# darren-huang/SmartStartContinuous

Measured on NVIDIA B200. Metric: mpc_rollout_steps_per_s, higher is better.
Workload: dtype bf16 (tcgen05, fp32 accumulate; first/last layer, state, scoring fp32)

## Files before the change

### smartstartcontinuous_b200/csrc/mpc_tc.cu

```cuda
#include <cuda_bf16.h>

#include <cstdlib>
#include <cstring>

#include "mpc_kernels.cuh"
#include "tc_ptx.cuh"
#include "tc_score_row.cuh"

namespace tc {

constexpr int TM = 128;
constexpr int NC = 128;
constexpr int NH = NC / 2;
constexpr int KSLAB = 256;
constexpr int STAGE_BYTES = NH * KSLAB * 2;
constexpr int NSTAGE = 4;
constexpr int K1_MAX = 32;
constexpr int ACC_SLOTS = 2;
constexpr int W1_CHUNK_BYTES_MAX = NH * K1_MAX * 2;
constexpr int A1_BYTES_MAX = TM * K1_MAX * 2;
constexpr int ROW_WARPS = 8;
constexpr int TPR = ROW_WARPS / 4;
constexpr int CPT = NC / TPR;
constexpr int ROW_THREADS = ROW_WARPS * 32;
constexpr int THREADS = ROW_THREADS + 64;
constexpr int HP_MAX = 512;
constexpr int MAX_DIN = (K1_MAX - 2) / 3;
__host__ __device__ constexpr int dz_of(int d) { return d <= 2 ? 2 : (d <= 3 ? 3 : (d <= 4 ? 4 : 8)); }
__host__ __device__ constexpr int k1_slots(int d, int da) { return 3 * (dz_of(d) + da) + 2 <= 16 ? 16 : 32; }
__host__ __device__ constexpr int w3_pair_floats(int dz) { return dz <= 2 ? 4 : (dz <= 4 ? 8 : 16); }
constexpr uint32_t TMEM_COLS = 512;
constexpr uint32_t COL_H1 = 0, COL_ACC = 256;
constexpr int CLUSTER = 2;

struct Params {
    const __nv_bfloat16* w1_img;
    const __nv_bfloat16* w2_img;
    const float* w3;
    const float* b3;
    int hp;
    int din;
    long long tile_begin, tile_end;
    int iters;
    unsigned long long* prof;
};

constexpr uint32_t IDESC = (1u << 4) | (1u << 7) | (1u << 10) | ((uint32_t)(NC >> 3) << 17) |
                           ((uint32_t)((2 * TM) >> 4) << 24);


#define TC_TRACE(ev)                                                                              \
    do {                                                                                          \
        if (p.prof && blockIdx.x == 0 && lane == 0 && trace_it == 0 && trace_t >= 10 && trace_t < 13) \
            trace_s[(trace_t - 10) * 256 + (ev)] = (unsigned long long)clock64();                  \
    } while (0)

template <int DZ>
struct SmemT {
    static constexpr size_t W2_RING = 0;
    static constexpr size_t W1 = W2_RING + (size_t)NSTAGE * STAGE_BYTES;
    static constexpr size_t A1 = W1 + (size_t)(HP_MAX / NC) * W1_CHUNK_BYTES_MAX;
    static constexpr size_t W3 = A1 + (size_t)A1_BYTES_MAX;
    static constexpr size_t ZX = W3 + (size_t)(HP_MAX / 2) * w3_pair_floats(DZ) * 4;
    static constexpr size_t BARS = ZX + (size_t)TPR * TM * 8 * 4;
    static constexpr int N_BARS = 3 * NSTAGE + 2 * ACC_SLOTS + 2 * (HP_MAX / NC) + 2;
    static constexpr size_t TMEM_PTR = BARS + (size_t)N_BARS * 8;
    static constexpr size_t TRACE = TMEM_PTR + 16;
    static constexpr size_t END = TRACE;
};

template <int DT, int DZ, int K1T>
__global__ void __launch_bounds__(THREADS, 1) mpc_rollout_tc_kernel(const RolloutArgs a, const Params p) {
    pdl_trigger();
    extern __shared__ __align__(128) unsigned char smem[];
    using Smem = SmemT<DZ>;
    constexpr int MAXIN = (K1T - 2) / 3;
    constexpr int W1_CHUNK_BYTES = NH * K1T * 2;
    constexpr int DZP = w3_pair_floats(DZ) / 2;
    unsigned char* w2_ring = smem + Smem::W2_RING;
    unsigned char* w1s = smem + Smem::W1;
    unsigned char* a1s = smem + Smem::A1;
    float* w3s = reinterpret_cast<float*>(smem + Smem::W3);
    float* zx = reinterpret_cast<float*>(smem + Smem::ZX);
    uint64_t* bars = reinterpret_cast<uint64_t*>(smem + Smem::BARS);
    uint64_t* w2_full = bars;
    uint64_t* w2_peer = w2_full + NSTAGE;
    uint64_t* w2_empty = w2_peer + NSTAGE;
    uint64_t* acc_full = w2_empty + NSTAGE;
    uint64_t* acc_free = acc_full + ACC_SLOTS;
    uint64_t* h1_ready = acc_free + ACC_SLOTS;
    uint64_t* l1_full = h1_ready + HP_MAX / NC;
    uint64_t* x_ready = l1_full + HP_MAX / NC;
    uint64_t* w1_full = x_ready + 1;
    uint32_t* tmem_ptr = reinterpret_cast<uint32_t*>(smem + Smem::TMEM_PTR);

    const int tid = threadIdx.x, warp = tid >> 5, lane = tid & 31;
    const int T = a.H + 1;
    unsigned long long* trace_s = reinterpret_cast<unsigned long long*>(smem + Smem::TRACE);
    if (p.prof && blockIdx.x == 0)
        for (int i = tid; i < 3 * 256; i += THREADS) trace_s[i] = 0;
    unsigned long long trace_clk0 = 0, trace_ns0 = 0;
    if (p.prof && blockIdx.x == 0 && tid == 0) {
        trace_clk0 = (unsigned long long)clock64();
        asm volatile("mov.u64 %0, %%globaltimer;" : "=l"(trace_ns0));
    }
    const int nch = p.hp / NC;
    const int nslab = p.hp / KSLAB;
    static_assert(KSLAB % NC == 0, "a K-slab covers whole layer-1 chunks");
    constexpr int CPS = KSLAB / NC;
    const uint32_t cta_rank = cluster_ctarank();
    const bool leader = cta_rank == 0;

    if (tid == 0) {
        for (int s = 0; s < NSTAGE; ++s) {
            mbar_init(&w2_full[s], leader ? 2 : 1);
            mbar_init(&w2_peer[s], 1);
            mbar_init(&w2_empty[s], 1);
        }
        for (int s = 0; s < ACC_SLOTS; ++s) { mbar_init(&acc_full[s], 1); mbar_init(&acc_free[s], 2 * ROW_WARPS); }
        for (int c = 0; c < HP_MAX / NC; ++c) { mbar_init(&h1_ready[c], 2 * ROW_WARPS); mbar_init(&l1_full[c], 1); }
        mbar_init(x_ready, 2 * 4);
        mbar_init(w1_full, 1);
        asm volatile("fence.mbarrier_init.release.cluster;" ::: "memory");
    }
    if (warp == 0) {
        asm volatile("tcgen05.alloc.cta_group::2.sync.aligned.shared::cta.b32 [%0], %1;" ::"r"(smem_u32(tmem_ptr)),
                     "n"(TMEM_COLS));
        asm volatile("tcgen05.relinquish_alloc_permit.cta_group::2.sync.aligned;");
    }
    for (int i = tid; i < (p.hp / 2) * (2 * DZP); i += THREADS) w3s[i] = p.w3[i];
    __syncthreads();
    if (tid == 0) {
        mbar_expect_tx(w1_full, (uint32_t)(nch * W1_CHUNK_BYTES));
        bulk_g2s(w1s, reinterpret_cast<const unsigned char*>(p.w1_img) + (size_t)cta_rank * nch * W1_CHUNK_BYTES,
                 (uint32_t)(nch * W1_CHUNK_BYTES), w1_full);
        mbar_wait<false>(w1_full, 0);
    }
    tc_fence_before();
    __syncthreads();
    cluster_sync_all();
    tc_fence_after();
    const uint32_t tmem = *tmem_ptr;

    if (warp < ROW_WARPS) {
        const int q = warp & 3, ch = warp >> 2;
        const int row = q * 32 + lane;
        const uint32_t lane_addr = tmem + ((uint32_t)(q * 32) << 16);
        uint32_t step_it = 0;
        float upd_s[DZ], upd_c[DZ];
#pragma unroll
        for (int j = 0; j < DZ; ++j) {
            upd_s[j] = j < a.d ? a.norm.std_z[j] : 0.f;
            upd_c[j] = j < a.d ? fmaf(__ldg(p.b3 + j), a.norm.std_z[j], a.norm.mean_z[j]) : 0.f;
            asm volatile("" : "+f"(upd_s[j]), "+f"(upd_c[j]));
        }
        for (int it = 0; it < p.iters; ++it) {
            const long long tile = p.tile_begin + (long long)it * gridDim.x + blockIdx.x;
            const long long k_local = tile * TM + row;
            const bool live = tile < p.tile_end && k_local < a.K_local;
            const long long n_qcols = 4 * ((a.K_local + TM - 1) / TM);
            const long long qcol = tile < p.tile_end ? tile * 4 + q : -1;
            float x[DT];
            ScoreAcc sc;
#pragma unroll
            for (int j = 0; j < DT; ++j) x[j] = j < a.d ? a.state0[j] : 0.f;
            if (ch == 1) score_init<DT>(a.plan, a.wp_index, x, sc);
            float act[SS_MAX_DA];
#pragma unroll
            for (int j = 0; j < SS_MAX_DA; ++j) act[j] = 0.f;
            ActionCursor cur;
            action_cursor_init(cur);
            if (ch == 0 && live) {
#pragma unroll
                for (int j = 0; j < SS_MAX_DA; ++j)
                    if (j < a.da) act[j] = fetch_action_seq(a.act, cur, k_local, a.k_offset + k_local, 0, j);
            }
            for (int t = 0; t < a.H; ++t, ++step_it) {
                const int trace_it = (warp == 0 || warp == 4) ? it : 1, trace_t = t;
                const int tb = warp == 4 ? 100 : 0;
                TC_TRACE(tb + 0);
                if (ch == 0) {
                    float xin[MAXIN];
#pragma unroll
                    for (int j = 0; j < MAXIN; ++j) xin[j] = 0.f;
#pragma unroll
                    for (int j = 0; j < DZ; ++j)
                        if (j < MAXIN) xin[j] = (x[j] - a.norm.mean_x[j]) * a.norm.inv_std_x[j];
#pragma unroll
                    for (int j = 0; j < SS_MAX_DA; ++j)
                        if (DZ + j < MAXIN) xin[DZ + j] = (act[j] - a.norm.mean_y[j]) * a.norm.inv_std_y[j];
                    float slot[K1T];
#pragma unroll
                    for (int s = 0; s < K1T; ++s) slot[s] = 0.f;
#pragma unroll
                    for (int j = 0; j < MAXIN; ++j) {
                        const float hi = bf16_hi(xin[j]);
                        const float lo = xin[j] - hi;
                        slot[3 * j] = hi;
                        slot[3 * j + 1] = hi;
                        slot[3 * j + 2] = lo;
                    }
                    slot[K1T - 2] = 1.f;
                    slot[K1T - 1] = 1.f;
#pragma unroll
                    for (int kc = 0; kc < K1T / 8; ++kc) {
                        uint4 v;
                        v.x = pack_bf16(slot[8 * kc], slot[8 * kc + 1]);
                        v.y = pack_bf16(slot[8 * kc + 2], slot[8 * kc + 3]);
                        v.z = pack_bf16(slot[8 * kc + 4], slot[8 * kc + 5]);
                        v.w = pack_bf16(slot[8 * kc + 6], slot[8 * kc + 7]);
                        *reinterpret_cast<uint4*>(a1s + kc * (TM * 16) + row * 16) = v;
                    }
                    TC_TRACE(60);
                    asm volatile("fence.proxy.async.shared::cta;" ::: "memory");
                    TC_TRACE(61);
                    __syncwarp();
                    if (lane == 0) mbar_arrive_leader(x_ready);
                }
                TC_TRACE(tb + 1);
                static_assert(CPT == 64, "two 32-column TMEM loads per thread and chunk");
                for (int c0 = 0; c0 < nch; c0 += 2) {
                    const uint32_t slot_i = (uint32_t)(c0 >> 1);
                    uint32_t v0[32], v1[32], pk0[16], pk1[16];
                    if (c0 == 0) mbar_wait<false>(&l1_full[0], step_it & 1);
                    TC_TRACE(tb + 2 + c0);
                    tc_fence_after();
                    tmem_ld32(lane_addr + COL_H1 + slot_i * NC + ch * CPT, v0);
                    tmem_ld32(lane_addr + COL_H1 + slot_i * NC + ch * CPT + 32, v1);
                    tmem_wait_ld();
                    asm volatile("bar.sync %0, 64;" ::"r"(2 + q) : "memory");
#pragma unroll
                    for (int c2 = 0; c2 < 16; ++c2) {
                        pk0[c2] = pack_bf16_relu(__uint_as_float(v0[2 * c2]), __uint_as_float(v0[2 * c2 + 1]));
                        pk1[c2] = pack_bf16_relu(__uint_as_float(v1[2 * c2]), __uint_as_float(v1[2 * c2 + 1]));
                    }
                    tmem_st16(lane_addr + COL_H1 + c0 * (NC / 2) + ch * (CPT / 2), pk0);
                    tmem_st16(lane_addr + COL_H1 + c0 * (NC / 2) + ch * (CPT / 2) + 16, pk1);
                    TC_TRACE(tb + 6 + c0);
                    if (c0 == 0) {
                        mbar_wait<false>(&l1_full[1], step_it & 1);
                        tc_fence_after();
                    }
                    TC_TRACE(tb + 3 + c0);
                    tmem_ld32(lane_addr + COL_ACC + slot_i * NC + ch * CPT, v0);
                    tmem_ld32(lane_addr + COL_ACC + slot_i * NC + ch * CPT + 32, v1);
                    tmem_wait_st();
                    tc_fence_before();
                    __syncwarp();
                    if (lane == 0) mbar_arrive_leader(&h1_ready[c0]);
                    tmem_wait_ld();
                    tc_fence_before();
                    __syncwarp();
                    if (lane == 0) mbar_arrive_leader(&acc_free[slot_i]);
#pragma unroll
                    for (int c2 = 0; c2 < 16; ++c2) {
                        pk0[c2] = pack_bf16_relu(__uint_as_float(v0[2 * c2]), __uint_as_float(v0[2 * c2 + 1]));
                        pk1[c2] = pack_bf16_relu(__uint_as_float(v1[2 * c2]), __uint_as_float(v1[2 * c2 + 1]));
                    }
                    tmem_st16(lane_addr + COL_H1 + (c0 + 1) * (NC / 2) + ch * (CPT / 2), pk0);
                    tmem_st16(lane_addr + COL_H1 + (c0 + 1) * (NC / 2) + ch * (CPT / 2) + 16, pk1);
                    tmem_wait_st();
                    tc_fence_before();
                    __syncwarp();
                    if (lane == 0) mbar_arrive_leader(&h1_ready[c0 + 1]);
                    TC_TRACE(tb + 7 + c0);
                }
                if (ch == 1) {
                    score_row<DT>(a, t, x, sc, live, k_local, qcol, n_qcols, lane);
                } else if (ch == 0 && live && t + 1 < a.H) {
                    TC_TRACE(70);
#pragma unroll
                    for (int j = 0; j < SS_MAX_DA; ++j)
                        if (j < a.da) act[j] = fetch_action_seq(a.act, cur, k_local, a.k_offset + k_local, t + 1, j);
                    TC_TRACE(71);
                }
                TC_TRACE(tb + 19);
                float2 zacc[DZ];
#pragma unroll
                for (int j = 0; j < DZ; ++j) zacc[j] = make_float2(0.f, 0.f);
                for (int n = 0; n < nch; ++n) {
                    const uint32_t slot_i = (uint32_t)(n & 1);
                    const uint32_t full_k = step_it * (uint32_t)((nch + 1 - (int)slot_i) >> 1) + (uint32_t)(n >> 1);
                    mbar_wait<false>(&acc_full[slot_i], full_k & 1);
                    TC_TRACE(tb + 10 + n);
                    tc_fence_after();
                    uint32_t v0[32], v1[32];
                    tmem_ld32(lane_addr + COL_ACC + slot_i * NC + ch * CPT, v0);
                    tmem_ld32(lane_addr + COL_ACC + slot_i * NC + ch * CPT + 32, v1);
                    tmem_wait_ld();
                    tc_fence_before();
                    __syncwarp();
                    if (lane == 0) mbar_arrive_leader(&acc_free[slot_i]);
                    const float* wrow = w3s + (size_t)((n * NC + ch * CPT) / 2) * (2 * DZP);
#pragma unroll
                    for (int j2 = 0; j2 < CPT / 2; ++j2) {
                        const uint32_t ua = j2 < 16 ? v0[(2 * j2) & 31] : v1[(2 * j2) & 31];
                        const uint32_t ub = j2 < 16 ? v0[(2 * j2 + 1) & 31] : v1[(2 * j2 + 1) & 31];
                        const float2 hh = make_float2(fmaxf(__uint_as_float(ua), 0.f), fmaxf(__uint_as_float(ub), 0.f));
                        const float* wp = wrow + j2 * (2 * DZP);
#pragma unroll
                        for (int jq = 0; jq < DZP / 2; ++jq) {
                            const float4 w = *reinterpret_cast<const float4*>(wp + 4 * jq);
                            if (2 * jq < DZ) zacc[2 * jq] = __ffma2_rn(hh, make_float2(w.x, w.y), zacc[2 * jq]);
                            if (2 * jq + 1 < DZ)
                                zacc[2 * jq + 1] = __ffma2_rn(hh, make_float2(w.z, w.w), zacc[2 * jq + 1]);
                        }
                    }
                    TC_TRACE(tb + 14 + n);
                }
#pragma unroll
                for (int j = 0; j < DZ; ++j) zx[(j * TPR + ch) * TM + row] = zacc[j].x + zacc[j].y;
                TC_TRACE(tb + 62);
                asm volatile("bar.sync %0, 64;" ::"r"(2 + q) : "memory");
                TC_TRACE(tb + 63);
#pragma unroll
                for (int j = 0; j < DZ; ++j) {
                    float zz = zx[(j * TPR) * TM + row];
#pragma unroll
                    for (int o = 1; o < TPR; ++o) zz += zx[(j * TPR + o) * TM + row];
                    x[j] += fmaf(zz, upd_s[j], upd_c[j]);
                }
                TC_TRACE(tb + 18);
            }
            if (ch == 1) {
                score_row<DT>(a, a.H, x, sc, live, k_local, qcol, n_qcols, lane);
                if (live && a.scores_out) a.scores_out[k_local] = sc.score;
            }
        }
    } else if (warp == ROW_WARPS) {
        if (leader) {
            uint32_t w2_it = 0, step_it = 0;
            const uint32_t l1_use[ACC_SLOTS] = {1 < nch ? 1u : 0u, 3 < nch ? 1u : 0u};
            const uint32_t use_per_step[ACC_SLOTS] = {l1_use[0] + (uint32_t)((nch + 1) >> 1),
                                                      l1_use[1] + (uint32_t)(nch >> 1)};
            const uint32_t a1_addr = smem_u32(a1s), w1_addr = smem_u32(w1s), ring_addr = smem_u32(w2_ring);
            constexpr int NCH_MAX = HP_MAX / NC;
            uint64_t l1_a[K1T / 16], l1_b[NCH_MAX][K1T / 16];
            uint32_t l1_d[NCH_MAX], l1_bar[NCH_MAX];
#pragma unroll
            for (int ks = 0; ks < K1T / 16; ++ks) {
                l1_a[ks] = make_desc(a1_addr + ks * 2 * (TM * 16), TM);
                asm volatile("" : "+l"(l1_a[ks]));
            }
#pragma unroll
            for (int c = 0; c < NCH_MAX; ++c) {
#pragma unroll
                for (int ks = 0; ks < K1T / 16; ++ks) {
                    l1_b[c][ks] = make_desc(w1_addr + c * W1_CHUNK_BYTES + ks * 2 * (NH * 16), NH);
                    asm volatile("" : "+l"(l1_b[c][ks]));
                }
                l1_d[c] = tmem + ((c & 1) ? COL_ACC : COL_H1) + (uint32_t)(c >> 1) * NC;
                l1_bar[c] = smem_u32(&l1_full[c]);
                asm volatile("" : "+r"(l1_d[c]), "+r"(l1_bar[c]));
            }
            for (int it = 0; it < p.iters; ++it) {
                for (int t = 0; t < a.H; ++t, ++step_it) {
                    const int trace_it = it, trace_t = t;
                    if (l1_use[1])
                        mbar_wait2(&acc_free[0], ((step_it * use_per_step[0]) & 1) ^ 1, &acc_free[1],
                                   ((step_it * use_per_step[1]) & 1) ^ 1);
                    else if (l1_use[0])
                        mbar_wait<true>(&acc_free[0], ((step_it * use_per_step[0]) & 1) ^ 1);
                    mbar_wait<true>(&w2_full[w2_it % NSTAGE], (w2_it / NSTAGE) & 1);
                    mbar_wait<true>(x_ready, step_it & 1);
                    TC_TRACE(20);
                    tc_fence_after();
                    if (elect_one()) {
#pragma unroll
                        for (int c = 0; c < NCH_MAX; ++c)
                            if (c < nch) {
#pragma unroll
                                for (int ks = 0; ks < K1T / 16; ++ks) umma2_ss(l1_d[c], l1_a[ks], l1_b[c][ks], IDESC, ks);
                                if (c == 0) tc_commit_pair_addr(l1_bar[0]);
                                else if (c == nch - 1) tc_commit_pair_addr(l1_bar[1]);
                            }
                    }
                    __syncwarp();
                    TC_TRACE(21);
                    for (int n = 0; n < nch; ++n) {
                        const uint32_t slot_i = (uint32_t)(n & 1);
                        const uint32_t free_k = slot_i ? step_it * use_per_step[1] + l1_use[1] + (uint32_t)(n >> 1)
                                                       : step_it * use_per_step[0] + l1_use[0] + (uint32_t)(n >> 1);
                        if (n == 0 || nslab < 1) mbar_wait<true>(&acc_free[slot_i], (free_k & 1) ^ 1);
                        else mbar_wait2(&acc_free[slot_i], (free_k & 1) ^ 1, &w2_full[w2_it % NSTAGE], (w2_it / NSTAGE) & 1);
                        TC_TRACE(41 + n);
                        for (int ksl = 0; ksl < nslab; ++ksl, ++w2_it) {
                            const uint32_t st = w2_it % NSTAGE;
                            const uint32_t d_tmem = tmem + COL_ACC + slot_i * NC;
                            const uint32_t a_tmem = tmem + COL_H1 + ksl * (KSLAB / 2);
                            const uint64_t b0 = make_desc(ring_addr + st * STAGE_BYTES, NH);
                            if (n == 0) {
                                static_assert(CPS == 2, "two layer-1 chunks per K-slab");
                                if (ksl > 0)
                                    mbar_wait2(&w2_full[st], (w2_it / NSTAGE) & 1, &h1_ready[ksl * CPS], step_it & 1);
                                else if (l1_use[0] == 0)
                                    mbar_wait<true>(&h1_ready[0], step_it & 1);
                                TC_TRACE(45 + 2 * ksl);
                                tc_fence_after();
                                if (elect_one()) {
#pragma unroll
                                    for (int ks = 0; ks < KSLAB / 32; ++ks)
                                        umma2_ts(d_tmem, a_tmem + ks * 8, b0 + (uint64_t)((ks * 2 * (NH * 16)) >> 4), IDESC,
                                                 (ksl | ks) != 0);
                                }
                                __syncwarp();
                                mbar_wait<true>(&h1_ready[ksl * CPS + 1], step_it & 1);
                                TC_TRACE(46 + 2 * ksl);
                                tc_fence_after();
                                if (elect_one()) {
#pragma unroll
                                    for (int ks = KSLAB / 32; ks < KSLAB / 16; ++ks)
                                        umma2_ts(d_tmem, a_tmem + ks * 8, b0 + (uint64_t)((ks * 2 * (NH * 16)) >> 4), IDESC, 1u);
                                    tc_commit_pair(&w2_empty[st]);
                                    if (ksl == nslab - 1) tc_commit_pair(&acc_full[slot_i]);
                                }
                            } else {
                                if (ksl > 0) mbar_wait<true>(&w2_full[st], (w2_it / NSTAGE) & 1);
                                tc_fence_after();
                                if (elect_one()) {
#pragma unroll
                                    for (int ks = 0; ks < KSLAB / 16; ++ks)
                                        umma2_ts(d_tmem, a_tmem + ks * 8, b0 + (uint64_t)((ks * 2 * (NH * 16)) >> 4), IDESC,
                                                 (ksl | ks) != 0);
                                    tc_commit_pair(&w2_empty[st]);
                                    if (ksl == nslab - 1) tc_commit_pair(&acc_full[slot_i]);
                                }
                            }
                            __syncwarp();
                            TC_TRACE(25 + n * 4 + ksl);
                        }
                    }
                }
            }
        } else {
            if (lane == 0) {
                uint32_t w2_it = 0;
                const long long total = (long long)p.iters * a.H * nch * nslab;
                for (long long i = 0; i < total; ++i, ++w2_it) {
                    const uint32_t st = w2_it % NSTAGE;
                    mbar_wait<false>(&w2_full[st], (w2_it / NSTAGE) & 1);
                    mbar_arrive_leader(&w2_full[st]);
                }
            }
        }
    } else {
        if (lane == 0) {
            uint32_t w2_it = 0;
            const int blocks = nch * nslab;
            for (int it = 0; it < p.iters; ++it)
                for (int t = 0; t < a.H; ++t)
                    for (int blk = 0; blk < blocks; ++blk, ++w2_it) {
                        const uint32_t st = w2_it % NSTAGE;
                        mbar_wait<false>(&w2_empty[st], ((w2_it / NSTAGE) & 1) ^ 1);
                        mbar_expect_tx(&w2_full[st], STAGE_BYTES);
                        bulk_g2s(w2_ring + (size_t)st * STAGE_BYTES,
                                 reinterpret_cast<const unsigned char*>(p.w2_img) +
                                     ((size_t)blk * CLUSTER + cta_rank) * STAGE_BYTES,
                                 STAGE_BYTES, &w2_full[st]);
                    }
        }
    }
    tc_fence_before();
    __syncthreads();
    cluster_sync_all();
    tc_fence_after();
    if (p.prof && blockIdx.x == 0) {
        for (int i = tid; i < 3 * 256; i += THREADS) p.prof[i] = trace_s[i];
        if (tid == 0) {
            unsigned long long ns1;
            asm volatile("mov.u64 %0, %%globaltimer;" : "=l"(ns1));
            p.prof[3 * 256] = (unsigned long long)clock64() - trace_clk0;
            p.prof[3 * 256 + 1] = ns1 - trace_ns0;
        }
    }
    if (warp == 0)
        asm volatile("tcgen05.dealloc.cta_group::2.sync.aligned.b32 %0, %1;" ::"r"(tmem), "n"(TMEM_COLS));
}

static uint16_t bf16_bits(float f) {
    uint32_t u;
    std::memcpy(&u, &f, 4);
    if ((u & 0x7fffffffu) > 0x7f800000u) return (uint16_t)((u >> 16) | 0x40);
    u += 0x7fffu + ((u >> 16) & 1u);
    return (uint16_t)(u >> 16);
}
static float bf16_val(uint16_t b) {
    uint32_t u = (uint32_t)b << 16;
    float f;
    std::memcpy(&f, &u, 4);
    return f;
}

static size_t smem_bytes(int d) {
    const int dz = dz_of(d);
    return (dz == 2 ? SmemT<2>::END : (dz <= 4 ? SmemT<4>::END : SmemT<8>::END)) + 128;
}

}

bool mpc_tc_shape_supported(const ss_ctx* c) {
    return c->L == 2 && c->h >= 64 && c->h + 2 <= tc::HP_MAX && c->d <= 8 && tc::dz_of(c->d) + c->da <= tc::MAX_DIN;
}

int mpc_tc_prepare(ss_ctx* c) {
    using namespace tc;
    const int h = c->h, d = c->d, din = c->d + c->da;
    const int k1 = k1_slots(d, c->da), dz = dz_of(d);
    const int W1_CHUNK_BYTES = NH * k1 * 2;
    const int hp = (h + 2 + KSLAB - 1) / KSLAB * KSLAB;
    const int nch = hp / NC, nslab = hp / KSLAB;
    const std::vector<double>&W1 = c->hw[0], &W2 = c->hw[1], &W3 = c->hw[2];
    const std::vector<double>&B1 = c->hb[0], &B2 = c->hb[1];
    std::vector<uint16_t> w1((size_t)CLUSTER * nch * (W1_CHUNK_BYTES / 2), 0);
    auto w1_at = [&](int slot, int u) -> uint16_t& {
        const int cidx = u / NC, r = (u % NC) / NH, nn = u % NH;
        return w1[((size_t)r * nch + cidx) * (W1_CHUNK_BYTES / 2) + (slot / 8) * (NH * 8) + nn * 8 + (slot % 8)];
    };
    for (int u = 0; u < h; ++u) {
        for (int j = 0; j < din; ++j) {
            const float w = (float)W1[(size_t)j * h + u];
            const uint16_t hi = bf16_bits(w), lo = bf16_bits(w - bf16_val(hi));
            const int in = j < d ? j : dz + (j - d);
            w1_at(3 * in, u) = hi;
            w1_at(3 * in + 1, u) = lo;
            w1_at(3 * in + 2, u) = hi;
        }
        const float b = (float)B1[u];
        const uint16_t hi = bf16_bits(b), lo = bf16_bits(b - bf16_val(hi));
        w1_at(k1 - 2, u) = hi;
        w1_at(k1 - 1, u) = lo;
    }
    w1_at(k1 - 2, h) = bf16_bits(1.f);
    w1_at(k1 - 2, h + 1) = bf16_bits(1.f);
    std::vector<uint16_t> w2((size_t)nch * nslab * CLUSTER * (STAGE_BYTES / 2), 0);
    auto w2_at = [&](int k, int u) -> uint16_t& {
        const int n = u / NC, r = (u % NC) / NH, nn = u % NH, ksl = k / KSLAB, kk = k % KSLAB;
        return w2[(((size_t)n * nslab + ksl) * CLUSTER + r) * (STAGE_BYTES / 2) + (kk / 8) * (NH * 8) + nn * 8 +
                  (kk % 8)];
    };
    for (int u = 0; u < h; ++u) {
        for (int k = 0; k < h; ++k) w2_at(k, u) = bf16_bits((float)W2[(size_t)k * h + u]);
        const float b = (float)B2[u];
        const uint16_t hi = bf16_bits(b), lo = bf16_bits(b - bf16_val(hi));
        w2_at(h, u) = hi;
        w2_at(h + 1, u) = lo;
    }
    const int dzp = w3_pair_floats(dz) / 2;
    std::vector<float> w3((size_t)hp * dzp, 0.f);
    for (int u = 0; u < h; ++u)
        for (int j = 0; j < d; ++j) w3[((size_t)(u / 2) * dzp + j) * 2 + (u & 1)] = (float)W3[(size_t)u * d + j];
    SS_CUDA_CHECK(c, c->tc_w1.ensure(w1.size() * 2));
    SS_CUDA_CHECK(c, c->tc_w2.ensure(w2.size() * 2));
    SS_CUDA_CHECK(c, c->tc_w3.ensure(w3.size() * 4));
    float b3[SS_MAX_D] = {};
    for (int j = 0; j < d; ++j) b3[j] = (float)c->hb[2][j];
    SS_CUDA_CHECK(c, c->tc_b3.ensure(SS_MAX_D * 4));
    SS_CUDA_CHECK(c, cudaMemcpyAsync(c->tc_b3.p, b3, SS_MAX_D * 4, cudaMemcpyHostToDevice, c->stream));
    SS_CUDA_CHECK(c, cudaMemcpyAsync(c->tc_w1.p, w1.data(), w1.size() * 2, cudaMemcpyHostToDevice, c->stream));
    SS_CUDA_CHECK(c, cudaMemcpyAsync(c->tc_w2.p, w2.data(), w2.size() * 2, cudaMemcpyHostToDevice, c->stream));
    SS_CUDA_CHECK(c, cudaMemcpyAsync(c->tc_w3.p, w3.data(), w3.size() * 4, cudaMemcpyHostToDevice, c->stream));
    SS_CUDA_CHECK(c, cudaStreamSynchronize(c->stream));
    c->tc_hp = hp;
    c->tc_ready = true;
    return SS_OK;
}

int mpc_tc_tile_rows() { return tc::TM; }

void mpc_tc_geometry(const ss_ctx* c, int* k1, int* dz, int* hp, int* NC_, int* NH_, int* KSLAB_, int* CLUSTER_,
                     int* dzp) {
    *k1 = tc::k1_slots(c->d, c->da);
    *dz = tc::dz_of(c->d);
    *hp = c->tc_hp;
    *NC_ = tc::NC; *NH_ = tc::NH; *KSLAB_ = tc::KSLAB; *CLUSTER_ = tc::CLUSTER;
    *dzp = tc::w3_pair_floats(tc::dz_of(c->d)) / 2;
}

int mpc_tc_grid(const ss_ctx* c, long long tiles) {
    const long long up = (tiles + tc::CLUSTER - 1) / tc::CLUSTER * tc::CLUSTER;
    const long long cap = c->sm_count / tc::CLUSTER * tc::CLUSTER;
    return (int)(up < cap ? up : cap);
}

int mpc_tc_launch(ss_ctx* c, const RolloutArgs& a, int* grid_blocks_out, long long tile_begin, long long tile_count) {
    using namespace tc;
    if (!c->tc_ready) SS_FAIL(c, SS_EUNSUPPORTED, "mpc: tcgen05 kernel not prepared for this model");
    Params p;
    std::memset(&p, 0, sizeof(p));
    p.w1_img = c->tc_w1.as<__nv_bfloat16>();
    p.w2_img = c->tc_w2.as<__nv_bfloat16>();
    p.w3 = c->tc_w3.as<float>();
    p.b3 = c->tc_b3.as<float>();
    p.hp = c->tc_hp;
    p.din = c->d + c->da;
    const long long all_tiles = (a.K_local + TM - 1) / TM;
    if (tile_count < 0) tile_count = all_tiles - tile_begin;
    if (tile_begin < 0 || tile_count < 1 || tile_begin + tile_count > all_tiles)
        SS_FAIL(c, SS_EINVAL, "mpc: tile range outside the batch");
    p.tile_begin = tile_begin;
    p.tile_end = tile_begin + tile_count;
    p.prof = nullptr;
    if (getenv("SS_TC_TRACE")) {
        SS_CUDA_CHECK(c, c->tc_misc.ensure((3 * 256 + 2) * 8));
        SS_CUDA_CHECK(c, cudaMemsetAsync(c->tc_misc.p, 0, (3 * 256 + 2) * 8, c->stream));
        p.prof = c->tc_misc.as<unsigned long long>();
    }
    const int grid = mpc_tc_grid(c, tile_count);
    if (grid_blocks_out) *grid_blocks_out = grid;
    p.iters = (int)((tile_count + grid - 1) / grid);
    const size_t smem = smem_bytes(a.d) + (p.prof ? 3 * 256 * 8 : 0);
    cudaLaunchConfig_t cfg;
    std::memset(&cfg, 0, sizeof(cfg));
    cfg.gridDim = dim3(grid);
    cfg.blockDim = dim3(THREADS);
    cfg.dynamicSmemBytes = smem;
    cfg.stream = c->stream;
    cudaLaunchAttribute attr[1];
    attr[0].id = cudaLaunchAttributeClusterDimension;
    attr[0].val.clusterDim.x = CLUSTER;
    attr[0].val.clusterDim.y = 1;
    attr[0].val.clusterDim.z = 1;
    cfg.attrs = attr;
    cfg.numAttrs = 1;
    cudaError_t e;
    const int dz = dz_of(a.d), k1 = k1_slots(a.d, a.da);
#define TC_LAUNCH(DT_, DZ_, K1_)                                                                              \
    do {                                                                                                      \
        e = cudaFuncSetAttribute(mpc_rollout_tc_kernel<DT_, DZ_, K1_>, cudaFuncAttributeMaxDynamicSharedMemorySize, \
                                 (int)smem);                                                                  \
        if (e == cudaSuccess) e = cudaLaunchKernelEx(&cfg, mpc_rollout_tc_kernel<DT_, DZ_, K1_>, a, p);       \
    } while (0)
    if (dz == 2 && k1 == 16) TC_LAUNCH(4, 2, 16);
    else if (dz == 3 && k1 == 16) TC_LAUNCH(4, 3, 16);
    else if (dz <= 4) TC_LAUNCH(4, 4, 32);
    else TC_LAUNCH(8, 8, 32);
#undef TC_LAUNCH
    if (e == cudaSuccess) e = cudaGetLastError();
    c->launches++;
    SS_CUDA_CHECK(c, e);
    if (p.prof) {
        std::vector<unsigned long long> h(3 * 256 + 2);
        SS_CUDA_CHECK(c, cudaMemcpyAsync(h.data(), p.prof, h.size() * 8, cudaMemcpyDeviceToHost, c->stream));
        SS_CUDA_CHECK(c, cudaStreamSynchronize(c->stream));
        fprintf(stderr, "[trace] block 0: %llu clk in %llu ns = %.0f MHz delivered SM clock\n", h[3 * 256], h[3 * 256 + 1],
                h[3 * 256 + 1] ? 1e3 * (double)h[3 * 256] / (double)h[3 * 256 + 1] : 0.0);
        for (int st2 = 0; st2 < 3; ++st2) {
            const unsigned long long* ev = &h[st2 * 256];
            const unsigned long long t0 = ev[0];
            fprintf(stderr, "[trace step %d] row: xsplit_done %llu | L1 full", 10 + st2, ev[1] - t0);
            for (int c2 = 0; c2 < 4; ++c2) fprintf(stderr, " %llu", ev[2 + c2] - t0);
            fprintf(stderr, " | L1 epi_done");
            for (int c2 = 0; c2 < 4; ++c2) fprintf(stderr, " %llu", ev[6 + c2] - t0);
            fprintf(stderr, " | L2 full");
            for (int c2 = 0; c2 < 4; ++c2) fprintf(stderr, " %llu", ev[10 + c2] - t0);
            fprintf(stderr, " | L2 epi_done");
            for (int c2 = 0; c2 < 4; ++c2) fprintf(stderr, " %llu", ev[14 + c2] - t0);
            fprintf(stderr, " | step_end %llu\n", ev[18] - t0);
            fprintf(stderr, "[trace step %d] detail: slots_stored %llu fence_done %llu | zx_stored %llu (ch1 %llu) bar_done %llu (ch1 %llu) | prefetch %llu .. %llu\n",
                    10 + st2, ev[60] - t0, ev[61] - t0, ev[62] - t0, ev[162] - t0, ev[63] - t0, ev[163] - t0, ev[70] - t0, ev[71] - t0);
            fprintf(stderr, "[trace step %d] mma: x_ready %llu | L1 issued", 10 + st2, ev[20] - t0);
            for (int c2 = 0; c2 < 4; ++c2) fprintf(stderr, " %llu", ev[21 + c2] - t0);
            fprintf(stderr, " | L2 slab issued");
            for (int c2 = 0; c2 < 16; ++c2) fprintf(stderr, " %llu", ev[25 + c2] - t0);
            fprintf(stderr, " | acc_free seen");
            for (int c2 = 0; c2 < 4; ++c2) fprintf(stderr, " %llu", ev[41 + c2] - t0);
            fprintf(stderr, " | n=0: h1_ready chunk0 %llu chunk1 %llu chunk2 %llu chunk3 %llu", ev[45] - t0, ev[46] - t0,
                    ev[47] - t0, ev[48] - t0);
            fprintf(stderr, "\n[trace step %d] ch1: L1 epi_done %llu | score_done %llu | L2 full", 10 + st2, ev[109] - t0, ev[119] - t0);
            for (int c2 = 0; c2 < 4; ++c2) fprintf(stderr, " %llu", ev[110 + c2] - t0);
            fprintf(stderr, " | L2 epi_done");
            for (int c2 = 0; c2 < 4; ++c2) fprintf(stderr, " %llu", ev[114 + c2] - t0);
            fprintf(stderr, " | ch0 prefetch_done %llu\n", ev[19] - t0);
        }
    }
    return SS_OK;
}
```

Before: 2.696 billion.

## Drain first two layer-1 chunks together before signaling layer-2 start

The layer-1 commit barrier l1_bar[0] now fires after chunks 0 and 1, and the epilogue drains both chunks (COL_H1 slot 0 and COL_ACC slot 0) in one block before arriving on h1_ready[0] and h1_ready[1] together. The MMA warp waits on acc_free[0] and h1_ready[1] jointly for the first slab instead of interleaving separate waits. This cuts barrier round-trips and fences per step at the start of layer 2. In exchange, the first layer-2 MMA cannot start until both chunks are converted, which reduces overlap between the epilogue and the tensor core.

After: 2.712 billion, median of 6. No clear change (+0.6%).

```diff
diff --git a/smartstartcontinuous_b200/csrc/mpc_tc.cu b/smartstartcontinuous_b200/csrc/mpc_tc.cu
--- a/smartstartcontinuous_b200/csrc/mpc_tc.cu
+++ b/smartstartcontinuous_b200/csrc/mpc_tc.cu
@@ -219,10 +219,50 @@
                 }
                 TC_TRACE(tb + 1);
                 static_assert(CPT == 64, "two 32-column TMEM loads per thread and chunk");
-                for (int c0 = 0; c0 < nch; c0 += 2) {
+                {
+                    uint32_t v0[32], v1[32], pa0[16], pa1[16], pk0[16], pk1[16];
+                    mbar_wait<false>(&l1_full[0], step_it & 1);
+                    TC_TRACE(tb + 2);
+                    tc_fence_after();
+                    tmem_ld32(lane_addr + COL_ACC + ch * CPT, v0);
+                    tmem_ld32(lane_addr + COL_ACC + ch * CPT + 32, v1);
+                    tmem_wait_ld();
+                    tc_fence_before();
+                    __syncwarp();
+                    if (lane == 0) mbar_arrive_leader(&acc_free[0]);
+#pragma unroll
+                    for (int c2 = 0; c2 < 16; ++c2) {
+                        pa0[c2] = pack_bf16_relu(__uint_as_float(v0[2 * c2]), __uint_as_float(v0[2 * c2 + 1]));
+                        pa1[c2] = pack_bf16_relu(__uint_as_float(v1[2 * c2]), __uint_as_float(v1[2 * c2 + 1]));
+                    }
+                    TC_TRACE(tb + 3);
+                    tmem_ld32(lane_addr + COL_H1 + ch * CPT, v0);
+                    tmem_ld32(lane_addr + COL_H1 + ch * CPT + 32, v1);
+                    tmem_wait_ld();
+                    asm volatile("bar.sync %0, 64;" ::"r"(2 + q) : "memory");
+#pragma unroll
+                    for (int c2 = 0; c2 < 16; ++c2) {
+                        pk0[c2] = pack_bf16_relu(__uint_as_float(v0[2 * c2]), __uint_as_float(v0[2 * c2 + 1]));
+                        pk1[c2] = pack_bf16_relu(__uint_as_float(v1[2 * c2]), __uint_as_float(v1[2 * c2 + 1]));
+                    }
+                    tmem_st16(lane_addr + COL_H1 + ch * (CPT / 2), pk0);
+                    tmem_st16(lane_addr + COL_H1 + ch * (CPT / 2) + 16, pk1);
+                    tmem_st16(lane_addr + COL_H1 + (NC / 2) + ch * (CPT / 2), pa0);
+                    tmem_st16(lane_addr + COL_H1 + (NC / 2) + ch * (CPT / 2) + 16, pa1);
+                    tmem_wait_st();
+                    tc_fence_before();
+                    __syncwarp();
+                    if (lane == 0) {
+                        mbar_arrive_leader(&h1_ready[0]);
+                        mbar_arrive_leader(&h1_ready[1]);
+                    }
+                    TC_TRACE(tb + 6);
+                    TC_TRACE(tb + 7);
+                }
+                for (int c0 = 2; c0 < nch; c0 += 2) {
                     const uint32_t slot_i = (uint32_t)(c0 >> 1);
                     uint32_t v0[32], v1[32], pk0[16], pk1[16];
-                    if (c0 == 0) mbar_wait<false>(&l1_full[0], step_it & 1);
+                    if (c0 == 2) mbar_wait<false>(&l1_full[1], step_it & 1);
                     TC_TRACE(tb + 2 + c0);
                     tc_fence_after();
                     tmem_ld32(lane_addr + COL_H1 + slot_i * NC + ch * CPT, v0);
@@ -237,10 +277,6 @@
                     tmem_st16(lane_addr + COL_H1 + c0 * (NC / 2) + ch * (CPT / 2), pk0);
                     tmem_st16(lane_addr + COL_H1 + c0 * (NC / 2) + ch * (CPT / 2) + 16, pk1);
                     TC_TRACE(tb + 6 + c0);
-                    if (c0 == 0) {
-                        mbar_wait<false>(&l1_full[1], step_it & 1);
-                        tc_fence_after();
-                    }
                     TC_TRACE(tb + 3 + c0);
                     tmem_ld32(lane_addr + COL_ACC + slot_i * NC + ch * CPT, v0);
                     tmem_ld32(lane_addr + COL_ACC + slot_i * NC + ch * CPT + 32, v1);
@@ -371,8 +407,8 @@
                             if (c < nch) {
 #pragma unroll
                                 for (int ks = 0; ks < K1T / 16; ++ks) umma2_ss(l1_d[c], l1_a[ks], l1_b[c][ks], IDESC, ks);
-                                if (c == 0) tc_commit_pair_addr(l1_bar[0]);
-                                else if (c == nch - 1) tc_commit_pair_addr(l1_bar[1]);
+                                if (c == 1) tc_commit_pair_addr(l1_bar[0]);
+                                if (c == nch - 1) tc_commit_pair_addr(l1_bar[1]);
                             }
                     }
                     __syncwarp();
@@ -381,7 +417,8 @@
                         const uint32_t slot_i = (uint32_t)(n & 1);
                         const uint32_t free_k = slot_i ? step_it * use_per_step[1] + l1_use[1] + (uint32_t)(n >> 1)
                                                        : step_it * use_per_step[0] + l1_use[0] + (uint32_t)(n >> 1);
-                        if (n == 0 || nslab < 1) mbar_wait<true>(&acc_free[slot_i], (free_k & 1) ^ 1);
+                        if (n == 0) mbar_wait2(&acc_free[0], (free_k & 1) ^ 1, &h1_ready[1], step_it & 1);
+                        else if (nslab < 1) mbar_wait<true>(&acc_free[slot_i], (free_k & 1) ^ 1);
                         else mbar_wait2(&acc_free[slot_i], (free_k & 1) ^ 1, &w2_full[w2_it % NSTAGE], (w2_it / NSTAGE) & 1);
                         TC_TRACE(41 + n);
                         for (int ksl = 0; ksl < nslab; ++ksl, ++w2_it) {
@@ -393,8 +430,6 @@
                                 static_assert(CPS == 2, "two layer-1 chunks per K-slab");
                                 if (ksl > 0)
                                     mbar_wait2(&w2_full[st], (w2_it / NSTAGE) & 1, &h1_ready[ksl * CPS], step_it & 1);
-                                else if (l1_use[0] == 0)
-                                    mbar_wait<true>(&h1_ready[0], step_it & 1);
                                 TC_TRACE(45 + 2 * ksl);
                                 tc_fence_after();
                                 if (elect_one()) {
@@ -404,7 +439,7 @@
                                                  (ksl | ks) != 0);
                                 }
                                 __syncwarp();
-                                mbar_wait<true>(&h1_ready[ksl * CPS + 1], step_it & 1);
+                                if (ksl > 0) mbar_wait<true>(&h1_ready[ksl * CPS + 1], step_it & 1);
                                 TC_TRACE(46 + 2 * ksl);
                                 tc_fence_after();
                                 if (elect_one()) {
```

## Reschedule TMEM accumulator slots so layer-2 chunk 0 overlaps layer-1 epilogue

Applied to the files above, without the earlier changes.

Reassigns which TMEM accumulator slot each layer-1 odd chunk and each layer-2 output chunk uses. Layer-2 chunk 0 now goes into slot 1, and the last layer-1 chunk (3) is issued later, only after the first layer-2 K-slab. The point is to let the layer-2 MMAs start before the row warps have drained every layer-1 accumulator, so MMA issue overlaps the epilogue better. The row-warp epilogue now waits per odd chunk on a separate l1_full barrier (three barriers instead of two). A constexpr simulator checks the mbarrier parities; the more complex ordering risks stalls or deadlock if the analysis misses a case.

Measured after the change: 2.752 billion before, 2.771 billion after (median of 6 runs). No clear change (+0.7%).

```diff
diff --git a/smartstartcontinuous_b200/csrc/mpc_tc.cu b/smartstartcontinuous_b200/csrc/mpc_tc.cu
--- a/smartstartcontinuous_b200/csrc/mpc_tc.cu
+++ b/smartstartcontinuous_b200/csrc/mpc_tc.cu
@@ -32,6 +32,59 @@
 constexpr uint32_t TMEM_COLS = 512;
 constexpr uint32_t COL_H1 = 0, COL_ACC = 256;
 constexpr int CLUSTER = 2;
+
+struct SlotUse {
+    int slot, k;
+};
+__host__ __device__ constexpr SlotUse slot_use(int nch, bool layer2, int c) {
+    return !layer2 ? SlotUse{0, c >> 1} : ((c & 1) ? SlotUse{0, nch / 2 + (c >> 1)} : SlotUse{1, c >> 1});
+}
+__host__ __device__ constexpr int slot_uses_per_step(int nch, int s) { return s == 0 ? nch : nch / 2; }
+__host__ __device__ constexpr uint32_t acc_free_parity(int nch, uint32_t step_it, bool layer2, int c) {
+    return ((step_it * (uint32_t)slot_uses_per_step(nch, slot_use(nch, layer2, c).slot) +
+             (uint32_t)slot_use(nch, layer2, c).k) & 1u) ^ 1u;
+}
+__host__ __device__ constexpr uint32_t acc_full_parity(int nch, uint32_t step_it, int n) {
+    return (step_it * (uint32_t)(nch / 2) + (uint32_t)(n >> 1)) & 1u;
+}
+__host__ __device__ constexpr bool slot_schedule_ok(int nch, int nsteps) {
+    constexpr int MAXU = 64;
+    int issued[2][MAXU] = {}, drained[2][MAXU] = {};
+    int n_iss[2] = {0, 0}, n_dr[2] = {0, 0}, full[2] = {0, 0};
+    for (int step = 0; step < nsteps; ++step) {
+        const uint32_t s_it = (uint32_t)step;
+        int seq[8] = {}, len = 0;
+        seq[len++] = 1;
+        seq[len++] = 100;
+        if (nch > 2) seq[len++] = 3;
+        for (int n = 1; n < nch; ++n) seq[len++] = 100 + n;
+        for (int i = 0; i < len; ++i) {
+            const bool l2 = seq[i] >= 100;
+            const int c = l2 ? seq[i] - 100 : seq[i];
+            const SlotUse u = slot_use(nch, l2, c);
+            const int g = n_iss[u.slot];
+            if (g >= MAXU || (uint32_t)g != s_it * (uint32_t)slot_uses_per_step(nch, u.slot) + (uint32_t)u.k) return false;
+            if (acc_free_parity(nch, s_it, l2, c) != (g == 0 ? 1u : (uint32_t)((g - 1) & 1))) return false;
+            issued[u.slot][n_iss[u.slot]++] = seq[i];
+            if (l2) {
+                if (acc_full_parity(nch, s_it, c) != (uint32_t)(full[u.slot] & 1)) return false;
+                ++full[u.slot];
+            }
+        }
+        for (int c = 1; c < nch; c += 2) drained[slot_use(nch, false, c).slot][n_dr[slot_use(nch, false, c).slot]++] = c;
+        for (int n = 0; n < nch; ++n) drained[slot_use(nch, true, n).slot][n_dr[slot_use(nch, true, n).slot]++] = 100 + n;
+        for (int s = 0; s < 2; ++s)
+            if (n_iss[s] != (step + 1) * slot_uses_per_step(nch, s) || full[s] != (step + 1) * (nch / 2)) return false;
+    }
+    for (int s = 0; s < 2; ++s) {
+        if (n_iss[s] != n_dr[s]) return false;
+        for (int i = 0; i < n_iss[s]; ++i)
+            if (issued[s][i] != drained[s][i]) return false;
+    }
+    return true;
+}
+static_assert(slot_schedule_ok(2, 7) && slot_schedule_ok(4, 7), "accumulator-slot parities");
+static_assert(slot_use(4, true, 0).slot == 1 && slot_use(4, false, 3).slot == 0, "layer-2 chunk 0 in slot 1");
 
 struct Params {
     const __nv_bfloat16* w1_img;
@@ -220,13 +273,13 @@
                 TC_TRACE(tb + 1);
                 static_assert(CPT == 64, "two 32-column TMEM loads per thread and chunk");
                 for (int c0 = 0; c0 < nch; c0 += 2) {
-                    const uint32_t slot_i = (uint32_t)(c0 >> 1);
+                    const uint32_t odd_col = COL_ACC + (uint32_t)slot_use(nch, false, c0 + 1).slot * NC;
                     uint32_t v0[32], v1[32], pk0[16], pk1[16];
                     if (c0 == 0) mbar_wait<false>(&l1_full[0], step_it & 1);
                     TC_TRACE(tb + 2 + c0);
                     tc_fence_after();
-                    tmem_ld32(lane_addr + COL_H1 + slot_i * NC + ch * CPT, v0);
-                    tmem_ld32(lane_addr + COL_H1 + slot_i * NC + ch * CPT + 32, v1);
+                    tmem_ld32(lane_addr + COL_H1 + (uint32_t)(c0 >> 1) * NC + ch * CPT, v0);
+                    tmem_ld32(lane_addr + COL_H1 + (uint32_t)(c0 >> 1) * NC + ch * CPT + 32, v1);
                     tmem_wait_ld();
                     asm volatile("bar.sync %0, 64;" ::"r"(2 + q) : "memory");
 #pragma unroll
@@ -237,21 +290,19 @@
                     tmem_st16(lane_addr + COL_H1 + c0 * (NC / 2) + ch * (CPT / 2), pk0);
                     tmem_st16(lane_addr + COL_H1 + c0 * (NC / 2) + ch * (CPT / 2) + 16, pk1);
                     TC_TRACE(tb + 6 + c0);
-                    if (c0 == 0) {
-                        mbar_wait<false>(&l1_full[1], step_it & 1);
-                        tc_fence_after();
-                    }
-                    TC_TRACE(tb + 3 + c0);
-                    tmem_ld32(lane_addr + COL_ACC + slot_i * NC + ch * CPT, v0);
-                    tmem_ld32(lane_addr + COL_ACC + slot_i * NC + ch * CPT + 32, v1);
                     tmem_wait_st();
                     tc_fence_before();
                     __syncwarp();
                     if (lane == 0) mbar_arrive_leader(&h1_ready[c0]);
+                    mbar_wait<false>(&l1_full[1 + (c0 >> 1)], step_it & 1);
+                    tc_fence_after();
+                    TC_TRACE(tb + 3 + c0);
+                    tmem_ld32(lane_addr + odd_col + ch * CPT, v0);
+                    tmem_ld32(lane_addr + odd_col + ch * CPT + 32, v1);
                     tmem_wait_ld();
                     tc_fence_before();
                     __syncwarp();
-                    if (lane == 0) mbar_arrive_leader(&acc_free[slot_i]);
+                    if (lane == 0) mbar_arrive_leader(&acc_free[slot_use(nch, false, c0 + 1).slot]);
 #pragma unroll
                     for (int c2 = 0; c2 < 16; ++c2) {
                         pk0[c2] = pack_bf16_relu(__uint_as_float(v0[2 * c2]), __uint_as_float(v0[2 * c2 + 1]));
@@ -279,9 +330,8 @@
 #pragma unroll
                 for (int j = 0; j < DZ; ++j) zacc[j] = make_float2(0.f, 0.f);
                 for (int n = 0; n < nch; ++n) {
-                    const uint32_t slot_i = (uint32_t)(n & 1);
-                    const uint32_t full_k = step_it * (uint32_t)((nch + 1 - (int)slot_i) >> 1) + (uint32_t)(n >> 1);
-                    mbar_wait<false>(&acc_full[slot_i], full_k & 1);
+                    const uint32_t slot_i = (uint32_t)slot_use(nch, true, n).slot;
+                    mbar_wait<false>(&acc_full[slot_i], acc_full_parity(nch, step_it, n));
                     TC_TRACE(tb + 10 + n);
                     tc_fence_after();
                     uint32_t v0[32], v1[32];
@@ -330,13 +380,10 @@
     } else if (warp == ROW_WARPS) {
         if (leader) {
             uint32_t w2_it = 0, step_it = 0;
-            const uint32_t l1_use[ACC_SLOTS] = {1 < nch ? 1u : 0u, 3 < nch ? 1u : 0u};
-            const uint32_t use_per_step[ACC_SLOTS] = {l1_use[0] + (uint32_t)((nch + 1) >> 1),
-                                                      l1_use[1] + (uint32_t)(nch >> 1)};
             const uint32_t a1_addr = smem_u32(a1s), w1_addr = smem_u32(w1s), ring_addr = smem_u32(w2_ring);
             constexpr int NCH_MAX = HP_MAX / NC;
             uint64_t l1_a[K1T / 16], l1_b[NCH_MAX][K1T / 16];
-            uint32_t l1_d[NCH_MAX], l1_bar[NCH_MAX];
+            uint32_t l1_d[NCH_MAX], l1_bar[3];
 #pragma unroll
             for (int ks = 0; ks < K1T / 16; ++ks) {
                 l1_a[ks] = make_desc(a1_addr + ks * 2 * (TM * 16), TM);
@@ -349,40 +396,41 @@
                     l1_b[c][ks] = make_desc(w1_addr + c * W1_CHUNK_BYTES + ks * 2 * (NH * 16), NH);
                     asm volatile("" : "+l"(l1_b[c][ks]));
                 }
-                l1_d[c] = tmem + ((c & 1) ? COL_ACC : COL_H1) + (uint32_t)(c >> 1) * NC;
-                l1_bar[c] = smem_u32(&l1_full[c]);
-                asm volatile("" : "+r"(l1_d[c]), "+r"(l1_bar[c]));
-            }
+                l1_d[c] = tmem + ((c & 1) ? COL_ACC + (uint32_t)slot_use(NCH_MAX, false, c).slot * NC
+                                          : COL_H1 + (uint32_t)(c >> 1) * NC);
+                asm volatile("" : "+r"(l1_d[c]));
+            }
+#pragma unroll
+            for (int i = 0; i < 3; ++i) {
+                l1_bar[i] = smem_u32(&l1_full[i]);
+                asm volatile("" : "+r"(l1_bar[i]));
+            }
+            auto l1_chunk = [&](int c) {
+#pragma unroll
+                for (int ks = 0; ks < K1T / 16; ++ks) umma2_ss(l1_d[c], l1_a[ks], l1_b[c][ks], IDESC, ks);
+            };
             for (int it = 0; it < p.iters; ++it) {
                 for (int t = 0; t < a.H; ++t, ++step_it) {
                     const int trace_it = it, trace_t = t;
-                    if (l1_use[1])
-                        mbar_wait2(&acc_free[0], ((step_it * use_per_step[0]) & 1) ^ 1, &acc_free[1],
-                                   ((step_it * use_per_step[1]) & 1) ^ 1);
-                    else if (l1_use[0])
-                        mbar_wait<true>(&acc_free[0], ((step_it * use_per_step[0]) & 1) ^ 1);
-                    mbar_wait<true>(&w2_full[w2_it % NSTAGE], (w2_it / NSTAGE) & 1);
+                    mbar_wait2(&acc_free[0], acc_free_parity(nch, step_it, false, 1), &w2_full[w2_it % NSTAGE],
+                               (w2_it / NSTAGE) & 1);
                     mbar_wait<true>(x_ready, step_it & 1);
                     TC_TRACE(20);
                     tc_fence_after();
                     if (elect_one()) {
-#pragma unroll
-                        for (int c = 0; c < NCH_MAX; ++c)
-                            if (c < nch) {
-#pragma unroll
-                                for (int ks = 0; ks < K1T / 16; ++ks) umma2_ss(l1_d[c], l1_a[ks], l1_b[c][ks], IDESC, ks);
-                                if (c == 0) tc_commit_pair_addr(l1_bar[0]);
-                                else if (c == nch - 1) tc_commit_pair_addr(l1_bar[1]);
-                            }
+                        l1_chunk(0);
+                        tc_commit_pair_addr(l1_bar[0]);
+                        l1_chunk(1);
+                        if (nch > 2) l1_chunk(2);
+                        tc_commit_pair_addr(l1_bar[1]);
                     }
                     __syncwarp();
                     TC_TRACE(21);
                     for (int n = 0; n < nch; ++n) {
-                        const uint32_t slot_i = (uint32_t)(n & 1);
-                        const uint32_t free_k = slot_i ? step_it * use_per_step[1] + l1_use[1] + (uint32_t)(n >> 1)
-                                                       : step_it * use_per_step[0] + l1_use[0] + (uint32_t)(n >> 1);
-                        if (n == 0 || nslab < 1) mbar_wait<true>(&acc_free[slot_i], (free_k & 1) ^ 1);
-                        else mbar_wait2(&acc_free[slot_i], (free_k & 1) ^ 1, &w2_full[w2_it % NSTAGE], (w2_it / NSTAGE) & 1);
+                        const uint32_t slot_i = (uint32_t)slot_use(nch, true, n).slot;
+                        if (n > 0)
+                            mbar_wait2(&acc_free[slot_i], acc_free_parity(nch, step_it, true, n), &w2_full[w2_it % NSTAGE],
+                                       (w2_it / NSTAGE) & 1);
                         TC_TRACE(41 + n);
                         for (int ksl = 0; ksl < nslab; ++ksl, ++w2_it) {
                             const uint32_t st = w2_it % NSTAGE;
@@ -393,8 +441,9 @@
                                 static_assert(CPS == 2, "two layer-1 chunks per K-slab");
                                 if (ksl > 0)
                                     mbar_wait2(&w2_full[st], (w2_it / NSTAGE) & 1, &h1_ready[ksl * CPS], step_it & 1);
-                                else if (l1_use[0] == 0)
-                                    mbar_wait<true>(&h1_ready[0], step_it & 1);
+                                else
+                                    mbar_wait2(&h1_ready[0], step_it & 1, &acc_free[slot_i],
+                                               acc_free_parity(nch, step_it, true, 0));
                                 TC_TRACE(45 + 2 * ksl);
                                 tc_fence_after();
                                 if (elect_one()) {
@@ -404,6 +453,18 @@
                                                  (ksl | ks) != 0);
                                 }
                                 __syncwarp();
+                                TC_TRACE(49 + 3 * ksl);
+                                if (ksl == 0 && nch > 2) {
+                                    mbar_wait<true>(&acc_free[0], acc_free_parity(nch, step_it, false, 3));
+                                    TC_TRACE(50);
+                                    tc_fence_after();
+                                    if (elect_one()) {
+                                        l1_chunk(3);
+                                        tc_commit_pair_addr(l1_bar[2]);
+                                    }
+                                    __syncwarp();
+                                    TC_TRACE(51);
+                                }
                                 mbar_wait<true>(&h1_ready[ksl * CPS + 1], step_it & 1);
                                 TC_TRACE(46 + 2 * ksl);
                                 tc_fence_after();
@@ -658,14 +719,14 @@
             fprintf(stderr, " | step_end %llu\n", ev[18] - t0);
             fprintf(stderr, "[trace step %d] detail: slots_stored %llu fence_done %llu | zx_stored %llu (ch1 %llu) bar_done %llu (ch1 %llu) | prefetch %llu .. %llu\n",
                     10 + st2, ev[60] - t0, ev[61] - t0, ev[62] - t0, ev[162] - t0, ev[63] - t0, ev[163] - t0, ev[70] - t0, ev[71] - t0);
-            fprintf(stderr, "[trace step %d] mma: x_ready %llu | L1 issued", 10 + st2, ev[20] - t0);
-            for (int c2 = 0; c2 < 4; ++c2) fprintf(stderr, " %llu", ev[21 + c2] - t0);
-            fprintf(stderr, " | L2 slab issued");
-            for (int c2 = 0; c2 < 16; ++c2) fprintf(stderr, " %llu", ev[25 + c2] - t0);
-            fprintf(stderr, " | acc_free seen");
-            for (int c2 = 0; c2 < 4; ++c2) fprintf(stderr, " %llu", ev[41 + c2] - t0);
-            fprintf(stderr, " | n=0: h1_ready chunk0 %llu chunk1 %llu chunk2 %llu chunk3 %llu", ev[45] - t0, ev[46] - t0,
-                    ev[47] - t0, ev[48] - t0);
+            fprintf(stderr, "[trace step %d] mma: x_ready %llu | L1 0-2 issued %llu | L2 slab issued", 10 + st2, ev[20] - t0,
+                    ev[21] - t0);
+            for (int c2 = 0; c2 < 8; ++c2) fprintf(stderr, " %llu", ev[25 + (c2 >> 1) * 4 + (c2 & 1)] - t0);
+            fprintf(stderr, " | acc_free seen n=1..3");
+            for (int c2 = 1; c2 < 4; ++c2) fprintf(stderr, " %llu", ev[41 + c2] - t0);
+            fprintf(stderr, " | n=0: h1_ready[0]+slot1 %llu K0 issued %llu | slot0 free %llu L1 chunk 3 issued %llu | "
+                            "h1_ready[1] %llu | h1_ready[2] %llu K2 issued %llu | h1_ready[3] %llu",
+                    ev[45] - t0, ev[49] - t0, ev[50] - t0, ev[51] - t0, ev[46] - t0, ev[47] - t0, ev[52] - t0, ev[48] - t0);
             fprintf(stderr, "\n[trace step %d] ch1: L1 epi_done %llu | score_done %llu | L2 full", 10 + st2, ev[109] - t0, ev[119] - t0);
             for (int c2 = 0; c2 < 4; ++c2) fprintf(stderr, " %llu", ev[110 + c2] - t0);
             fprintf(stderr, " | L2 epi_done");
```
